# NVlabs/curobo

Measured on NVIDIA B200. Metric: rollout_cost_grad_evals_per_sec, higher is better.
Workload: dtype f32

## Files before the change

### curobo_b200/csrc/cb200_blob.h

```cpp
#pragma once
#include <stdint.h>

namespace cb200 {

constexpr int32_t kBlobMagic = 0x30324243;
constexpr int kMaxLinks = 64;

struct BlobHeader {
  int32_t magic;
  int32_t total_bytes;
  int32_t smem_bytes;
  int32_t nl, D, S, L, P;
  int32_t n_levels;
  int32_t off_fixed;
  int32_t off_joff;
  int32_t off_link_map;
  int32_t off_joint_map;
  int32_t off_joint_type;
  int32_t off_tool_map;
  int32_t off_spheres;
  int32_t off_sph_link;
  int32_t off_padding;
  int32_t off_link_sph_off;
  int32_t off_link_sph_idx;
  int32_t off_level_off;
  int32_t off_level_links;
  int32_t off_anc_mask;
  int32_t off_jl_off;
  int32_t off_jl_idx;
  int32_t off_limits;
  int32_t off_pairs;
  int32_t n_cl, n_lp;
  int32_t off_cl_link;
  int32_t off_cl_start;
  int32_t off_cl_bound;
  int32_t off_lp;
  int32_t n_fk_steps;
  int32_t off_fk_sched;
  int32_t off_cl_bound_scene;
  int32_t off_sph_cl;
  int32_t n_sphere_cfgs;
  int32_t reserved[10];
};
static_assert(sizeof(BlobHeader) == 192, "BlobHeader must be 192 bytes");

}
```

### curobo_b200/csrc/cb200_kernels.cu

```cuda
#include <cuda_runtime.h>
#include <stdio.h>
#include <stdlib.h>
#include <string.h>

#include <algorithm>
#include <cmath>
#include <vector>

#include "../../include/curobo_b200.h"
#include "cb200_blob.h"
#include "cb200_bspline.cuh"
#include "cb200_dynamics.cuh"
#include "cb200_dynamics_tile.cuh"
#include "cb200_launch.h"
#include "cb200_math.cuh"
#include "cb200_mesh.cuh"
#include "cb200_warp.cuh"

using namespace cb200;

namespace {

constexpr int kWarpsPerCta = 8;
#ifndef CB200_MINB
// ... 189 lines not shown
    pg[0] = pg[1] = pg[2] = pg[4] = pg[5] = pg[6] = 0.0f;
    if (do_pose) {
      const int gi = a.idxs_goal ? __ldg(a.idxs_goal + b) : 0;
      const bool term = !(h < a.H - 1 && a.H > 1);
      const float *axes = term ? a.pose_axes_t : a.pose_axes_nt;
      const float *tol = term ? a.pose_tol_t : a.pose_tol_nt;
      const size_t go = ((size_t)gi * L + t) * cfg.num_goalset;
      const PoseOut po = tool_pose_cost(p, qt, a.goal_position + go * 3, a.goal_quat + go * 4, cfg.num_goalset,
                                        cfg.pose_weight[0], cfg.pose_weight[1], axes, t,
                                        tol != nullptr ? __ldg(tol + 2 * t) : 0.0f,
                                        tol != nullptr ? __ldg(tol + 2 * t + 1) : 0.0f, cfg.pose_rotation_method);
      const V3 om = quat_grad_to_omega(qt, po.gq_w, po.gq_x, po.gq_y, po.gq_z);
      pg[0] = po.g_pos.x;
      pg[1] = po.g_pos.y;
      pg[2] = po.g_pos.z;
      pg[4] = om.x;
      pg[5] = om.y;
      pg[6] = om.z;
      pose_c += po.pos_cost + po.rot_cost;
      if (a.pose_cost) {
        a.pose_cost[((size_t)e * L + t) * 2] = po.pos_cost;
        a.pose_cost[((size_t)e * L + t) * 2 + 1] = po.rot_cost;
      }
      if (a.pose_goalset_idx) a.pose_goalset_idx[(size_t)e * L + t] = po.goal_idx;
    }
  }
  __syncwarp();
}

struct RowB1 {
  float self_c, fmax, scene_c;
  int bi, bj, nnz;
};

template <bool SWEEP, int SCENE, bool CULL2 = true>
__device__ __forceinline__ RowB1 row_phase_b1(const FusedArgs &a, const RobotView &rv, const EvalSmem &es, int lane, int e,
                                              int b, const float4 *prev_sph, const float4 *next_sph) {
  const cb200_rollout_cfg &cfg = a.cfg;
  const int S = rv.S;
  RowB1 r{0.0f, 0.0f, 0.0f, 0, 0, 0};
  if (cfg.self_weight > 0.0f && rv.P > 0) {
    r.fmax = (rv.n_lp > 0) ? warp_self_collision_tiles<true, CULL2>(rv, es, lane, r.bi, r.bj)
                           : warp_self_collision_pairs(es.gsph, rv.pairs, rv.P, lane, r.bi, r.bj);
    r.self_c = (r.fmax > 0.0f) ? 0.5f * cfg.self_weight * r.fmax : 0.0f;
  }
  if (a.self_cost && lane == 0) a.self_cost[e] = r.self_c;
  __syncwarp();
  const bool do_scene = SCENE != 0 && cfg.scene_weight > 0.0f;
  const int env = (a.env_query_idx != nullptr) ? __ldg(a.env_query_idx + b) : 0;
  const float sdt = (SWEEP && cfg.use_speed_metric && (a.dt != nullptr || a.spl.knots != nullptr))
                        ? (a.spl.knots != nullptr ? __ldg(a.spl.traj_dt + __ldg(a.spl.goal_idx)) : __ldg(a.dt))
                        : 0.0f;
  int ce = 0, ncub = 0;
  bool cull = false;
  if ((SCENE & 1) && do_scene) {
    ce = env < a.cuboids.num_envs ? env : 0;
    ncub = a.cuboids.count[ce];
    if (ncub > a.cuboids.max_n) ncub = a.cuboids.max_n;
    cull = !SWEEP && rv.n_lp > 0 && ncub <= 32;
    if (cull) {
#pragma unroll 1
      for (int ca = lane; ca < rv.n_cl; ca += 32) {
        const float4 cb = rv.cl_bound_scene[ca];
        uint32_t mask = 0u;
        if (cb.w >= 0.0f) {
          const float *Tk = es.cumul + 12 * rv.cl_link[ca];
          const V3 cw = mk3(Tk[0] * cb.x + Tk[1] * cb.y + Tk[2] * cb.z + Tk[3], Tk[4] * cb.x + Tk[5] * cb.y + Tk[6] * cb.z + Tk[7],
                            Tk[8] * cb.x + Tk[9] * cb.y + Tk[10] * cb.z + Tk[11]);
#pragma unroll 1
          for (int i = 0; i < ncub; ++i) {
            const int kk = ce * a.cuboids.max_n + i;
            if (a.cuboids.enable[kk] != 1) continue;
            const ObsFrame f = load_obs_frame(a.cuboids.inv_pose + 8 * kk);
            const SdfGrad sg = cuboid_sdf_grad(to_obstacle(f, cw), ldgf(a.cuboids.dims + 4 * kk), ldgf(a.cuboids.dims + 4 * kk + 1),
                                               ldgf(a.cuboids.dims + 4 * kk + 2));
            if (sg.sdf < cb.w + cfg.scene_activation) mask |= (1u << i);
          }
        }
        es.cmask[ca] = mask;
      }
      __syncwarp();
    }
  }
#pragma unroll 1
  for (int s = lane; s < S; s += 32) {
    V3 g = mk3(0, 0, 0);
    float c = 0.0f;
    if (do_scene) {
      const float4 sp = es.sph[s];
      const V3 cen = mk3(sp.x, sp.y, sp.z);
      if (!SWEEP) {
        if (sp.w >= 0.0f) {
          if (SCENE & 1) {
            uint32_t m = cull ? es.cmask[rv.sph_cl[s]] : 0xffffffffu;
            const float radj = sp.w + cfg.scene_activation;
#pragma unroll 1
            for (int i = 0; i < ncub && m != 0u; ++i) {
              if (cull && !((m >> i) & 1u)) continue;
              if (cull) m &= ~(1u << i);
              const int kk = ce * a.cuboids.max_n + i;
              if (a.cuboids.enable[kk] != 1) continue;
              const ObsFrame f = load_obs_frame(a.cuboids.inv_pose + 8 * kk);
              const SdfGrad sg = cuboid_sdf_grad(to_obstacle(f, cen), ldgf(a.cuboids.dims + 4 * kk), ldgf(a.cuboids.dims + 4 * kk + 1),
                                                 ldgf(a.cuboids.dims + 4 * kk + 2));
              const float pen = radj - sg.sdf;
              if (pen > 0.0f) {
                float ac, as;
                collision_activation(pen, cfg.scene_activation, ac, as);
                c += cfg.scene_weight * ac;
                g = g + (cfg.scene_weight * as) * from_obstacle(f, sg.n);
              }
            }
          }
          if (SCENE & 2) {
            const CuboidSet none{};
            c += sphere_scene_discrete<2>(cen, sp.w, cfg.scene_activation, cfg.scene_weight, none, a.voxels, env, g);
          }
        }
      } else {
        V3 pv = cen, nx = cen;
        if (prev_sph != nullptr) {
          const float4 t = prev_sph[s];
          pv = mk3(t.x, t.y, t.z);
        }
        if (next_sph != nullptr) {
          const float4 t = next_sph[s];
          nx = mk3(t.x, t.y, t.z);
        }
        c = sphere_scene_swept<SCENE>(cen, sp.w, cfg.scene_activation, cfg.scene_weight, prev_sph != nullptr, pv,
                                      next_sph != nullptr, nx, a.cuboids, a.voxels, env, g);
        if (cfg.use_speed_metric && prev_sph != nullptr && next_sph != nullptr) speed_metric(pv, cen, nx, sdt, c, g);
      }
    }
    es.gsph[s] = make_float4(g.x, g.y, g.z, 0.0f);
    r.nnz += (g.x != 0.0f || g.y != 0.0f || g.z != 0.0f) ? 1 : 0;
    r.scene_c += c;
    if (a.scene_cost) a.scene_cost[(size_t)e * S + s] = c;
  }
  __syncwarp();
  r.nnz = (int)__reduce_add_sync(kFull, (unsigned)r.nnz) + 2;
  return r;
}

template <bool SMALL = false>
__device__ __forceinline__ void row_phase_b2(const FusedArgs &a, const RobotView &rv, const EvalSmem &es,
                                             const unsigned char *smem_blob, int lane, int e, const RowB1 &r,
                                             float cs_cost, float pose_c) {
  if (r.fmax > 0.0f && lane == 0) {
    const float4 pi = es.sph[r.bi], pj = es.sph[r.bj];
    const float w = a.cfg.self_weight;
    float4 gi = es.gsph[r.bi], gj = es.gsph[r.bj];
    const float gx = w * (pj.x - pi.x), gy = w * (pj.y - pi.y), gz = w * (pj.z - pi.z);
    gi.x += gx;
    gi.y += gy;
    gi.z += gz;
    gj.x -= gx;
    gj.y -= gy;
    gj.z -= gz;
    es.gsph[r.bi] = gi;
    es.gsph[r.bj] = gj;
  }
  __syncwarp();
  float *gq = a.grad_q + (size_t)e * rv.D;
  if (!warp_fk_backward_sparse<SMALL>(rv, es, lane, gq, r.nnz)) warp_fk_backward_cold(smem_blob, a.blob, es.cumul, lane, gq);
  const float tot = warp_sum(cs_cost + pose_c + r.scene_c) + r.self_c;
  if (lane == 0) a.cost[e] = tot;
  __syncwarp();
}

#ifdef CB200_OOL_PHASES
struct PhaseAOut {
  float cs_cost, pose_c;
};
static __device__ __noinline__ PhaseAOut phase_a_ool(const FusedArgs *a, const unsigned char *smem, float *base, int lane,
                                                     int e, int b, int h) {
  const RobotView rv = make_robot_view(smem, a->blob);
  const EvalSmem es = carve_eval_smem(base, rv.nl, rv.D, rv.S, rv.L, rv.n_cl);
  PhaseAOut o;
  row_phase_a<false>(*a, rv, es, lane, e, b, h, o.cs_cost, o.pose_c);
  return o;
}
template <int SCENE>
static __device__ __noinline__ RowB1 phase_b1_ool(const FusedArgs *a, const unsigned char *smem, float *base, int lane, int e,
                                                  int b) {
  const RobotView rv = make_robot_view(smem, a->blob);
  const EvalSmem es = carve_eval_smem(base, rv.nl, rv.D, rv.S, rv.L, rv.n_cl);
  return row_phase_b1<false, SCENE>(*a, rv, es, lane, e, b, nullptr, nullptr);
}
static __device__ __noinline__ void phase_b2_ool(const FusedArgs *a, const unsigned char *smem, float *base, int lane, int e,
                                                 RowB1 r, float cs_cost, float pose_c) {
  const RobotView rv = make_robot_view(smem, a->blob);
  const EvalSmem es = carve_eval_smem(base, rv.nl, rv.D, rv.S, rv.L, rv.n_cl);
  row_phase_b2(*a, rv, es, smem, lane, e, r, cs_cost, pose_c);
}
#endif

template <int SCENE, bool SPLINE, int MINB = CB200_MINB>
__global__ void __launch_bounds__(kWarpsPerCta * 32, MINB) rollout_fused_kernel(const __grid_constant__ FusedArgs a) {
  CB200_EXTERN_SHARED __align__(128) unsigned char smem[];
  __shared__ unsigned long long mbar;
  stage_blob_to_smem(smem, a.blob, (uint32_t)a.blob_smem_bytes, &mbar);
  const int warp = threadIdx.x >> 5, lane = threadIdx.x & 31, nwarps = blockDim.x >> 5;
  float *base = reinterpret_cast<float *>(smem + a.blob_smem_bytes) + (size_t)warp * a.eval_floats;
  const int N = a.B * a.H;
  const int stride = gridDim.x * nwarps;
  int e = blockIdx.x * nwarps + warp;
  while (e < N) {
    int b = e, h = 0;
    if (a.H != 1) {
      b = e / a.H;
      h = e - b * a.H;
    }
#ifndef CB200_OOL_PHASES
    const RobotView rv = make_robot_view(smem, a.blob);
    const EvalSmem es = carve_eval_smem(base, rv.nl, rv.D, rv.S, rv.L, rv.n_cl);
    float cs_cost = 0.0f, pose_c = 0.0f;
    row_phase_a<SPLINE>(a, rv, es, lane, e, b, h, cs_cost, pose_c);
    const RowB1 r = row_phase_b1<false, SCENE, MINB != 3>(a, rv, es, lane, e, b, nullptr, nullptr);
    row_phase_b2<MINB == 3>(a, rv, es, smem, lane, e, r, cs_cost, pose_c);
#else
    const PhaseAOut pa = phase_a_ool(&a, smem, base, lane, e, b, h);
    const RowB1 r = phase_b1_ool<SCENE>(&a, smem, base, lane, e, b);
    phase_b2_ool(&a, smem, base, lane, e, r, pa.cs_cost, pa.pose_c);
#endif
    if (a.work_counter != nullptr) {
      int nxt = 0;
      if (lane == 0) nxt = stride + atomicAdd(a.work_counter, 1);
      e = __shfl_sync(kFull, nxt, 0);
    } else {
      e += stride;
    }
  }
  if (a.work_counter != nullptr && lane == 0) {
    __threadfence();
    if (atomicAdd(a.work_counter + 1, 1) == stride - 1) {
      a.work_counter[0] = 0;
      a.work_counter[1] = 0;
    }
  }
}

constexpr int kBigWarps = 16;

template <int SCENE, bool SMALL = false>
__device__ __forceinline__ RowB1 row_phase_b1_list(const FusedArgs &a, const RobotView &rv, const EvalSmem &es, int lane, int e,
                                                   int b, int &n_list, bool &dense) {
  const cb200_rollout_cfg &cfg = a.cfg;
  const int S = rv.S;
  RowB1 r{0.0f, 0.0f, 0.0f, 0, 0, 0};
  n_list = 0;
  dense = false;
  if (cfg.self_weight > 0.0f && rv.P > 0) {
    r.fmax = warp_self_collision_tiles<false, !SMALL>(rv, es, lane, r.bi, r.bj);
    r.self_c = (r.fmax > 0.0f) ? 0.5f * cfg.self_weight * r.fmax : 0.0f;
  }
  if (a.self_cost && lane == 0) a.self_cost[e] = r.self_c;
  __syncwarp();
  const bool do_scene = SCENE != 0 && cfg.scene_weight > 0.0f;
  const int env = (a.env_query_idx != nullptr) ? __ldg(a.env_query_idx + b) : 0;
  int ce = 0, ncub = 0;
  bool cull = false;
  if ((SCENE & 1) && do_scene) {
    ce = env < a.cuboids.num_envs ? env : 0;
    ncub = a.cuboids.count[ce];
    if (ncub > a.cuboids.max_n) ncub = a.cuboids.max_n;
    cull = rv.n_lp > 0 && ncub <= 32;
    if (cull) {
#pragma unroll 1
      for (int ca = lane; ca < rv.n_cl; ca += 32) {
        const float4 cb = rv.cl_bound_scene[ca];
        uint32_t mask = 0u;
        if (cb.w >= 0.0f) {
          const float *Tk = es.cumul + 12 * rv.cl_link[ca];
          const V3 cw = mk3(Tk[0] * cb.x + Tk[1] * cb.y + Tk[2] * cb.z + Tk[3], Tk[4] * cb.x + Tk[5] * cb.y + Tk[6] * cb.z + Tk[7],
                            Tk[8] * cb.x + Tk[9] * cb.y + Tk[10] * cb.z + Tk[11]);
#pragma unroll 1
          for (int i = 0; i < ncub; ++i) {
            const int kk = ce * a.cuboids.max_n + i;
            if (a.cuboids.enable[kk] != 1) continue;
            const ObsFrame f = load_obs_frame(a.cuboids.inv_pose + 8 * kk);
            const SdfGrad sg = cuboid_sdf_grad(to_obstacle(f, cw), ldgf(a.cuboids.dims + 4 * kk), ldgf(a.cuboids.dims + 4 * kk + 1),
                                               ldgf(a.cuboids.dims + 4 * kk + 2));
            if (sg.sdf < cb.w + cfg.scene_activation) mask |= (1u << i);
          }
        }
        es.cmask[ca] = mask;
      }
      __syncwarp();
    }
  }
  bool ft_live = false;
  const unsigned lt = (1u << lane) - 1u;
#pragma unroll 1
  for (int base = 0; base < S; base += 32) {
    const int s = base + lane;
    V3 g = mk3(0, 0, 0);
    float c = 0.0f;
// ... 2142 lines not shown
  h->S = S;
  h->L = L;
  h->P = P;
  h->n_levels = n_levels;
  h->off_fixed = take((int64_t)nl * 48);
  h->off_joff = take((int64_t)nl * 8);
  h->off_link_map = take((int64_t)nl * 2);
  h->off_joint_map = take((int64_t)nl * 2);
  h->off_joint_type = take(nl);
  h->off_tool_map = take((int64_t)L * 2);
  h->off_spheres = take((int64_t)S * 16);
  h->off_sph_link = take((int64_t)S * 2);
  h->off_padding = take((int64_t)S * 4);
  h->off_link_sph_off = take((int64_t)(nl + 1) * 2);
  h->off_link_sph_idx = take((int64_t)S * 2);
  h->off_level_off = take((int64_t)(nl + 1) * 2);
  h->off_level_links = take((int64_t)nl * 2);
  h->off_anc_mask = take((int64_t)nl * 8);
  h->off_jl_off = take((int64_t)(D + 1) * 2);
  h->off_jl_idx = take((int64_t)nl * 2);
  h->off_limits = take((int64_t)10 * D * 4);
  const int max_cl = std::min(nl, S);
  h->off_cl_link = take((int64_t)max_cl * 2);
  h->off_cl_start = take((int64_t)(max_cl + 1) * 2);
  h->off_cl_bound = take((int64_t)max_cl * 16);
  h->off_lp = take((int64_t)n_lp_cap * 4);
  h->off_fk_sched = take((int64_t)nl * 8);
  h->off_cl_bound_scene = take((int64_t)max_cl * 16);
  h->off_sph_cl = take((int64_t)S);
  h->smem_bytes = (int32_t)off;
  h->off_pairs = take((int64_t)P * 4);
  h->total_bytes = (int32_t)off;
  return off;
}

static int lp_cap(const cb200_robot_sizes *sz) {
  const int m = std::min(sz->num_links, sz->num_spheres);
  return std::min(m * (m - 1) / 2, std::max(sz->num_pairs, 0));
}

int cb200_voxel_mip_block(void) { return kMipBlock; }

int64_t cb200_voxel_mip_stride(const float *host_params, int num_layers) {
  if (host_params == nullptr || num_layers < 1) return -1;
  int64_t best = 1;
  for (int k = 0; k < num_layers; ++k) {
    const int64_t nx = (int64_t)host_params[4 * k], ny = (int64_t)host_params[4 * k + 1], nz = (int64_t)host_params[4 * k + 2];
    best = std::max(best, ((nx + kMipBlock - 1) >> kMipShift) * ((ny + kMipBlock - 1) >> kMipShift) * ((nz + kMipBlock - 1) >> kMipShift));
  }
  return best;
}

int cb200_voxel_build_mip(const cb200_voxel_set *vs, cb200_stream_t stream) {
  CB200_DEVICE_GUARD((vs != nullptr ? vs->mip : nullptr));
  if (vs == nullptr || vs->mip == nullptr || vs->mip_stride < 1 || vs->features == nullptr || vs->params == nullptr ||
      vs->max_n < 1 || vs->num_envs < 1)
    return ret(cudaErrorInvalidValue);
  const int n_layers = vs->max_n * vs->num_envs;
  const long long n = (long long)vs->mip_stride * n_layers;
  const int grid = (int)std::min<long long>((n + 127) / 128, 148LL * 16);
  CB200_LAUNCH(voxel_mip_kernel, grid, 128, 0, (cudaStream_t)stream, to_dev(vs), const_cast<uint16_t *>(vs->mip), n_layers);
  return launch_status();
}

int64_t cb200_robot_blob_bytes(const cb200_robot_sizes *sz) {
  BlobHeader h;
  return blob_layout(sz, nullptr, &h, lp_cap(sz));
}

int64_t cb200_pack_robot_blob(void *out, int64_t out_bytes, const cb200_robot_sizes *sz, const float *fixed_transforms,
                              const int16_t *link_map, const int16_t *joint_map, const int8_t *joint_map_type,
                              const float *joint_offset_map, const int16_t *tool_frame_map, const float *link_spheres,
                              const int16_t *link_sphere_map, const float *sphere_padding,
                              const int16_t *collision_pairs, const float *position_limits,
                              const float *velocity_limits, const float *acceleration_limits, const float *jerk_limits,
                              const float *effort_limits) {
  BlobHeader h;
  const int64_t total = blob_layout(sz, link_map, &h, lp_cap(sz));
  if (total < 0) return total;
  if (out_bytes < total) return -3;
  const int nl = h.nl, D = h.D, S = h.S, L = h.L, P = h.P;
  const int n_cfg = sz->num_sphere_configs > 1 ? sz->num_sphere_configs : 1;
  h.n_sphere_cfgs = n_cfg;
  unsigned char *o = static_cast<unsigned char *>(out);
  memset(o, 0, (size_t)total);
  memcpy(o, &h, sizeof(h));
  memcpy(o + h.off_fixed, fixed_transforms, (size_t)nl * 48);
  memcpy(o + h.off_joff, joint_offset_map, (size_t)nl * 8);
  memcpy(o + h.off_link_map, link_map, (size_t)nl * 2);
  memcpy(o + h.off_joint_map, joint_map, (size_t)nl * 2);
  memcpy(o + h.off_joint_type, joint_map_type, (size_t)nl);
  if (L) memcpy(o + h.off_tool_map, tool_frame_map, (size_t)L * 2);
  for (int l = 0; l < nl; ++l) {
    const int jt = joint_map_type[l];
    if (jt < -1 || jt > 5) return -4;
    if (jt >= 0 && (joint_map[l] < 0 || joint_map[l] >= D)) return -5;
  }
  for (int t = 0; t < L; ++t)
    if (tool_frame_map[t] < 0 || tool_frame_map[t] >= nl) return -6;
  if (S) {
    memcpy(o + h.off_spheres, link_spheres, (size_t)S * 16);
    memcpy(o + h.off_sph_link, link_sphere_map, (size_t)S * 2);
    memcpy(o + h.off_padding, sphere_padding, (size_t)S * 4);
  }
  int16_t *lso = reinterpret_cast<int16_t *>(o + h.off_link_sph_off);
  int16_t *lsi = reinterpret_cast<int16_t *>(o + h.off_link_sph_idx);
  int n = 0;
  for (int l = 0; l < nl; ++l) {
    lso[l] = (int16_t)n;
    for (int s = 0; s < S; ++s) {
      if (link_sphere_map[s] < 0 || link_sphere_map[s] >= nl) return -7;
      if (link_sphere_map[s] == l) lsi[n++] = (int16_t)s;
    }
  }
  lso[nl] = (int16_t)n;
  std::vector<int> depth(nl, 0);
  unsigned long long *anc = reinterpret_cast<unsigned long long *>(o + h.off_anc_mask);
  anc[0] = 1ull;
  for (int l = 1; l < nl; ++l) {
    depth[l] = depth[link_map[l]] + 1;
    anc[l] = anc[link_map[l]] | (1ull << l);
  }
  int16_t *lvo = reinterpret_cast<int16_t *>(o + h.off_level_off);
  int16_t *lvl = reinterpret_cast<int16_t *>(o + h.off_level_links);
  n = 0;
  for (int lev = 0; lev < h.n_levels; ++lev) {
    lvo[lev] = (int16_t)n;
    for (int l = 0; l < nl; ++l)
      if (depth[l] == lev) lvl[n++] = (int16_t)l;
  }
  lvo[h.n_levels] = (int16_t)n;
  {
    uint32_t *sched = reinterpret_cast<uint32_t *>(o + h.off_fk_sched);
    int steps = 0;
    for (int lev = 1; lev < h.n_levels; ++lev) {
      for (int i = lvo[lev]; i < lvo[lev + 1]; i += 2) {
        const uint32_t l0 = (uint32_t)lvl[i], p0 = (uint32_t)link_map[l0];
        sched[2 * steps] = (l0 * 48u) | ((p0 * 48u) << 16);
        sched[2 * steps + 1] = 0xffffu;
        if (i + 1 < lvo[lev + 1]) {
          const uint32_t l1 = (uint32_t)lvl[i + 1], p1 = (uint32_t)link_map[l1];
          sched[2 * steps + 1] = (l1 * 48u) | ((p1 * 48u) << 16);
        }
        ++steps;
      }
    }
    reinterpret_cast<BlobHeader *>(o)->n_fk_steps = steps;
  }
  int16_t *jlo = reinterpret_cast<int16_t *>(o + h.off_jl_off);
  int16_t *jli = reinterpret_cast<int16_t *>(o + h.off_jl_idx);
  n = 0;
  for (int d = 0; d < D; ++d) {
    jlo[d] = (int16_t)n;
    for (int l = 0; l < nl; ++l)
      if (joint_map_type[l] >= 0 && joint_map[l] == d) jli[n++] = (int16_t)l;
  }
  jlo[D] = (int16_t)n;
  float *lim = reinterpret_cast<float *>(o + h.off_limits);
  const float *srcs[5] = {position_limits, velocity_limits, acceleration_limits, jerk_limits, effort_limits};
  for (int k = 0; k < 5; ++k)
    for (int i = 0; i < 2 * D; ++i) lim[k * 2 * D + i] = srcs[k] ? srcs[k][i] : (i < D ? -1e30f : 1e30f);
  for (int p = 0; p < P; ++p) {
    const int i = collision_pairs[2 * p], j = collision_pairs[2 * p + 1];
    if (i < 0 || j < 0 || i >= S || j >= S) return -8;
  }
  if (P) memcpy(o + h.off_pairs, collision_pairs, (size_t)P * 4);
// ... 508 lines not shown
```

### curobo_b200/csrc/cb200_warp.cuh

```cuda
#pragma once
#include "cb200_blob.h"
#include "cb200_math.cuh"

namespace cb200 {

constexpr unsigned kFull = 0xffffffffu;

struct RobotView {
  int nl, D, S, L, P, n_levels;
  const float *fixed;
  const float *joff;
  const int16_t *link_map;
  const int16_t *joint_map;
  const int8_t *joint_type;
  const int16_t *tool_map;
  const float4 *spheres;
  const int16_t *sph_link;
  const float *padding;
  const int16_t *link_sph_off;
  const int16_t *link_sph_idx;
  const int16_t *level_off;
  const int16_t *level_links;
  const unsigned long long *anc_mask;
  const int16_t *jl_off;
  const int16_t *jl_idx;
  const float *limits;
  const uint32_t *pairs;
  int n_cl, n_lp;
  const int16_t *cl_link;
  const int16_t *cl_start;
  const float4 *cl_bound;
  const uint32_t *lp;
  int n_fk_steps;
  const uint32_t *fk_sched;
  const float4 *cl_bound_scene;
  const uint8_t *sph_cl;
};

__device__ __forceinline__ RobotView make_robot_view(const unsigned char *smem_blob, const unsigned char *gmem_blob) {
  const BlobHeader *h = reinterpret_cast<const BlobHeader *>(smem_blob);
  RobotView v;
  v.nl = h->nl;
  v.D = h->D;
  v.S = h->S;
  v.L = h->L;
  v.P = h->P;
  v.n_levels = h->n_levels;
  v.fixed = reinterpret_cast<const float *>(smem_blob + h->off_fixed);
  v.joff = reinterpret_cast<const float *>(smem_blob + h->off_joff);
  v.link_map = reinterpret_cast<const int16_t *>(smem_blob + h->off_link_map);
  v.joint_map = reinterpret_cast<const int16_t *>(smem_blob + h->off_joint_map);
  v.joint_type = reinterpret_cast<const int8_t *>(smem_blob + h->off_joint_type);
  v.tool_map = reinterpret_cast<const int16_t *>(smem_blob + h->off_tool_map);
  v.spheres = reinterpret_cast<const float4 *>(smem_blob + h->off_spheres);
  v.sph_link = reinterpret_cast<const int16_t *>(smem_blob + h->off_sph_link);
  v.padding = reinterpret_cast<const float *>(smem_blob + h->off_padding);
  v.link_sph_off = reinterpret_cast<const int16_t *>(smem_blob + h->off_link_sph_off);
  v.link_sph_idx = reinterpret_cast<const int16_t *>(smem_blob + h->off_link_sph_idx);
  v.level_off = reinterpret_cast<const int16_t *>(smem_blob + h->off_level_off);
  v.level_links = reinterpret_cast<const int16_t *>(smem_blob + h->off_level_links);
  v.anc_mask = reinterpret_cast<const unsigned long long *>(smem_blob + h->off_anc_mask);
  v.jl_off = reinterpret_cast<const int16_t *>(smem_blob + h->off_jl_off);
  v.jl_idx = reinterpret_cast<const int16_t *>(smem_blob + h->off_jl_idx);
  v.limits = reinterpret_cast<const float *>(smem_blob + h->off_limits);
  v.pairs = reinterpret_cast<const uint32_t *>(gmem_blob + h->off_pairs);
  v.n_cl = h->n_cl;
  v.n_lp = h->n_lp;
  v.cl_link = reinterpret_cast<const int16_t *>(smem_blob + h->off_cl_link);
  v.cl_start = reinterpret_cast<const int16_t *>(smem_blob + h->off_cl_start);
  v.cl_bound = reinterpret_cast<const float4 *>(smem_blob + h->off_cl_bound);
  v.lp = reinterpret_cast<const uint32_t *>(smem_blob + h->off_lp);
  v.n_fk_steps = h->n_fk_steps;
  v.fk_sched = reinterpret_cast<const uint32_t *>(smem_blob + h->off_fk_sched);
  v.cl_bound_scene = reinterpret_cast<const float4 *>(smem_blob + h->off_cl_bound_scene);
  v.sph_cl = reinterpret_cast<const uint8_t *>(smem_blob + h->off_sph_cl);
  return v;
}

struct EvalSmem {
  float *cumul;
  float4 *sph;
  float4 *gsph;
  float *ft;
  float *contrib;
  float *qv;
  float *gqv;
  float *pose_g;
  float4 *bc;
  uint32_t *cmask;
  float4 *glist;
};
__host__ __device__ inline int eval_smem_floats(int nl, int D, int S, int L, int n_cl) {
  int n = nl * 12 + S * 8 + nl * 8 + n_cl * 4;
  n += nl + D + D + L * 8 + n_cl;
  return (n + 3) & ~3;
}
__device__ __forceinline__ EvalSmem carve_eval_smem(float *base, int nl, int D, int S, int L, int n_cl) {
  EvalSmem e;
  e.cumul = base;
  e.sph = reinterpret_cast<float4 *>(base + nl * 12);
  e.gsph = e.sph + S;
  e.ft = base + nl * 12 + S * 8;
  e.bc = reinterpret_cast<float4 *>(e.ft + nl * 8);
  e.contrib = e.ft + nl * 8 + n_cl * 4;
  e.qv = e.contrib + nl;
  e.gqv = e.qv + D;
  e.pose_g = e.gqv + D;
  e.cmask = reinterpret_cast<uint32_t *>(e.pose_g + L * 8);
  e.glist = nullptr;
  return e;
}

constexpr int kGradListCap = 96;
__host__ __device__ inline int big_smem_floats(int nl, int D, int S, int L, int n_cl) {
  int n = nl * 12 + S * 4 + nl * 8 + n_cl * 4 + kGradListCap * 4;
  n += nl + D + D + L * 8 + n_cl;
  return (n + 3) & ~3;
}
__device__ __forceinline__ EvalSmem carve_big_smem(float *base, int nl, int D, int S, int L, int n_cl) {
  EvalSmem e;
  e.cumul = base;
  e.sph = reinterpret_cast<float4 *>(base + nl * 12);
  e.gsph = nullptr;
  e.ft = base + nl * 12 + S * 4;
  e.bc = reinterpret_cast<float4 *>(e.ft + nl * 8);
  e.glist = e.bc + n_cl;
  e.contrib = reinterpret_cast<float *>(e.glist + kGradListCap);
  e.qv = e.contrib + nl;
  e.gqv = e.qv + D;
  e.pose_g = e.gqv + D;
  e.cmask = reinterpret_cast<uint32_t *>(e.pose_g + L * 8);
  return e;
}

__device__ __forceinline__ float warp_sum(float v) {
#pragma unroll
  for (int o = 16; o > 0; o >>= 1) v += __shfl_xor_sync(kFull, v, o);
  return v;
}

__device__ __forceinline__ void warp_fk_compose(const RobotView &rv, const EvalSmem &es, int lane);
__device__ __forceinline__ void warp_fk(const RobotView &rv, const EvalSmem &es, int lane) {
  const bool scratch = rv.S * 4 >= rv.nl * 12;
  float *loc = scratch ? reinterpret_cast<float *>(es.sph) : es.cumul;
  #pragma unroll 1
  for (int l = lane; l < rv.nl; l += 32) {
    int jt = rv.joint_type[l];
    float th = 0.0f;
    if (jt >= 0) th = rv.joff[2 * l] * es.qv[rv.joint_map[l]] + rv.joff[2 * l + 1];
    local_link_transform(rv.fixed + 12 * l, jt, th, (l == 0 ? es.cumul : loc) + 12 * l);
  }
  __syncwarp();
  warp_fk_compose(rv, es, lane);
}

__device__ __forceinline__ void warp_fk_compose(const RobotView &rv, const EvalSmem &es, int lane) {
  const bool scratch = rv.S * 4 >= rv.nl * 12;
  const float *loc = scratch ? reinterpret_cast<const float *>(es.sph) : es.cumul;
  const int sub = lane >> 4, k = lane & 15;
  const bool lane_ok = k < 12;
  const uint32_t row_off = (uint32_t)(k >> 2) * 16u, col_off = (uint32_t)(k & 3) * 4u, k_off = (uint32_t)k * 4u;
  const float cw = ((k & 3) == 3) ? 1.0f : 0.0f;
  unsigned char *cumb = reinterpret_cast<unsigned char *>(es.cumul);
  const unsigned char *locb = reinterpret_cast<const unsigned char *>(loc);
#pragma unroll 1
  for (int st = 0; st < rv.n_fk_steps; ++st) {
    const uint32_t w = rv.fk_sched[2 * st + sub];
    const uint32_t l_off = w & 0xffffu, p_off = w >> 16;
    const bool act = lane_ok && (l_off != 0xffffu);
    float out = 0.0f;
    if (act) {
      const float4 pr = *reinterpret_cast<const float4 *>(cumb + p_off + row_off);
      const float *Lm = reinterpret_cast<const float *>(locb + l_off + col_off);
      out = pr.x * Lm[0] + pr.y * Lm[4] + pr.z * Lm[8] + cw * pr.w;
    }
    if (!scratch) __syncwarp();
    if (act) *reinterpret_cast<float *>(cumb + l_off + k_off) = out;
    __syncwarp();
  }
}

__device__ __forceinline__ void warp_spheres(const RobotView &rv, const EvalSmem &es, int lane, float4 *out_global,
                                             const float4 *cfg_spheres = nullptr) {
  #pragma unroll 1
  for (int s = lane; s < rv.S; s += 32) {
    const float *T = es.cumul + 12 * rv.sph_link[s];
    const float4 p = cfg_spheres != nullptr ? __ldg(cfg_spheres + s) : rv.spheres[s];
    const float4 r0 = *reinterpret_cast<const float4 *>(T), r1 = *reinterpret_cast<const float4 *>(T + 4),
                 r2 = *reinterpret_cast<const float4 *>(T + 8);
    float4 w;
    w.x = r0.x * p.x + r0.y * p.y + r0.z * p.z + r0.w;
    w.y = r1.x * p.x + r1.y * p.y + r1.z * p.z + r1.w;
    w.z = r2.x * p.x + r2.y * p.y + r2.z * p.z + r2.w;
    w.w = p.w;
    es.sph[s] = w;
    if (out_global != nullptr) out_global[s] = w;
    if (es.gsph != nullptr) {
      w.w = p.w + rv.padding[s];
      es.gsph[s] = w;
    }
  }
}

__device__ __forceinline__ float warp_self_collision_pairs(const float4 *psph, const uint32_t *pairs, int P, int lane,
                                                           int &bi, int &bj) {
  float best = 0.0f;
  uint32_t best_p = 0xffffffffu;
  #pragma unroll 1
  for (int p = lane; p < P; p += 32) {
    const uint32_t pr = __ldg(pairs + p);
    const float4 a = psph[pr & 0xffffu], b = psph[pr >> 16];
    const float rs = a.w + b.w;
    const float dx = a.x - b.x, dy = a.y - b.y, dz = a.z - b.z;
    float f = rs * rs - (dx * dx + dy * dy + dz * dz);
    if (!(a.w >= 0.0f && b.w >= 0.0f)) f = 0.0f;
    if (f > best) {
      best = f;
      best_p = (uint32_t)p;
    }
  }
  const uint32_t fb = __reduce_max_sync(kFull, __float_as_uint(best));
  const uint32_t cand = (__float_as_uint(best) == fb && best > 0.0f) ? best_p : 0xffffffffu;
  const uint32_t win = __reduce_min_sync(kFull, cand);
  bi = bj = 0;
  if (win == 0xffffffffu) return 0.0f;
  const uint32_t pr = __ldg(pairs + win);
  bi = (int)(pr & 0xffffu);
  bj = (int)(pr >> 16);
  return __uint_as_float(fb);
}

template <bool PADDED_COPY>
__device__ __forceinline__ float4 padded_sphere(const RobotView &rv, const EvalSmem &es, int i) {
  if (PADDED_COPY) return es.gsph[i];
  float4 x = es.sph[i];
  x.w += rv.padding[i];
  return x;
}

template <bool PADDED_COPY = true, bool CULL2 = true>
__device__ __forceinline__ float warp_self_collision_tiles(const RobotView &rv, const EvalSmem &es, int lane, int &bi,
                                                           int &bj, int base0 = 0, int stride = 32,
                                                           unsigned char *idx_scratch = nullptr,
                                                           unsigned long long *key_out = nullptr, bool fill_bounds = true) {
  if (fill_bounds) {
    #pragma unroll 1
    for (int a = lane; a < rv.n_cl; a += 32) {
      const float4 c = rv.cl_bound[a];
      const float *T = es.cumul + 12 * rv.cl_link[a];
      es.bc[a] = make_float4(T[0] * c.x + T[1] * c.y + T[2] * c.z + T[3], T[4] * c.x + T[5] * c.y + T[6] * c.z + T[7],
                             T[8] * c.x + T[9] * c.y + T[10] * c.z + T[11], c.w);
    }
    __syncwarp();
  }
  unsigned long long key = 0ull;
  #pragma unroll 1
  for (int base = base0; base < rv.n_lp; base += stride) {
    uint32_t pr = 0;
    bool hit = false;
    if (base + lane < rv.n_lp) {
      pr = rv.lp[base + lane];
      const float4 A = es.bc[pr & 0xffffu], B = es.bc[pr >> 16];
      const float dx = A.x - B.x, dy = A.y - B.y, dz = A.z - B.z, rs = A.w + B.w;
      hit = (A.w >= 0.0f) && (B.w >= 0.0f) && (dx * dx + dy * dy + dz * dz < rs * rs);
    }
    unsigned m = __ballot_sync(kFull, hit);
    while (m) {
      const int src = __ffs(m) - 1;
// ... 70 lines not shown
  bj = 0xffff - (int)(key & 0xffffu);
  return __uint_as_float((uint32_t)(key >> 32));
}

__device__ __forceinline__ void warp_fk_upsweep(const RobotView &rv, const EvalSmem &es, int lane, float *gq_out);
__device__ __forceinline__ void warp_fk_backward(const RobotView &rv, const EvalSmem &es, int lane, float *gq_out) {
  #pragma unroll 1
  for (int k = lane; k < rv.nl; k += 32) {
    const float *Tk = es.cumul + 12 * k;
    const V3 o = mk3(Tk[3], Tk[7], Tk[11]);
    V3 F = mk3(0, 0, 0), T = mk3(0, 0, 0);
    #pragma unroll 1
    for (int i = rv.link_sph_off[k]; i < rv.link_sph_off[k + 1]; ++i) {
      const int s = rv.link_sph_idx[i];
      const float4 g4 = es.gsph[s];
      const V3 g = mk3(g4.x, g4.y, g4.z);
      if (g.x == 0.0f && g.y == 0.0f && g.z == 0.0f) continue;
      const float4 p4 = es.sph[s];
      F = F + g;
      T = T + cross(mk3(p4.x, p4.y, p4.z) - o, g);
    }
    for (int e = 0; e < rv.L; ++e) {
      if (rv.tool_map[e] != k) continue;
      F = F + mk3(es.pose_g[8 * e + 0], es.pose_g[8 * e + 1], es.pose_g[8 * e + 2]);
      T = T + mk3(es.pose_g[8 * e + 4], es.pose_g[8 * e + 5], es.pose_g[8 * e + 6]);
    }
    float *ft = es.ft + 8 * k;
    ft[0] = F.x;
    ft[1] = F.y;
    ft[2] = F.z;
    ft[4] = T.x;
    ft[5] = T.y;
    ft[6] = T.z;
  }
  __syncwarp();
  warp_fk_upsweep(rv, es, lane, gq_out);
}

__device__ __forceinline__ void warp_fk_upsweep(const RobotView &rv, const EvalSmem &es, int lane, float *gq_out) {
  #pragma unroll 1
  for (int j = lane; j < rv.nl; j += 32) {
    const int jt = rv.joint_type[j];
    float res = 0.0f;
    if (jt >= 0) {
      const float *Tj = es.cumul + 12 * j;
      const V3 oj = mk3(Tj[3], Tj[7], Tj[11]);
      V3 F = mk3(0, 0, 0), T = mk3(0, 0, 0);
      #pragma unroll 1
      for (int k = j; k < rv.nl; ++k) {
        if (!((rv.anc_mask[k] >> j) & 1ull)) continue;
        const float *ft = es.ft + 8 * k;
        const V3 Fk = mk3(ft[0], ft[1], ft[2]);
        const float *Tk = es.cumul + 12 * k;
        const V3 ok = mk3(Tk[3], Tk[7], Tk[11]);
        F = F + Fk;
        T = T + mk3(ft[4], ft[5], ft[6]) + cross(ok - oj, Fk);
      }
      const int ax = (jt >= JT_XR) ? jt - JT_XR : jt;
      const V3 a = mk3(Tj[ax], Tj[4 + ax], Tj[8 + ax]);
      res = rv.joff[2 * j] * ((jt >= JT_XR) ? dot(a, T) : dot(a, F));
    }
    es.contrib[j] = res;
  }
  __syncwarp();
  for (int d = lane; d < rv.D; d += 32) {
    float g = es.gqv[d];
    for (int i = rv.jl_off[d]; i < rv.jl_off[d + 1]; ++i) g += es.contrib[rv.jl_idx[i]];
    gq_out[d] = g;
  }
}

static __device__ __noinline__ void warp_fk_backward_cold(const unsigned char *smem_blob, const unsigned char *gmem_blob,
                                                          float *eval_base, int lane, float *gq_out) {
  const RobotView rv = make_robot_view(smem_blob, gmem_blob);
  const EvalSmem es = carve_eval_smem(eval_base, rv.nl, rv.D, rv.S, rv.L, rv.n_cl);
  warp_fk_backward(rv, es, lane, gq_out);
}

template <bool SMALL = false>
__device__ __forceinline__ bool warp_fk_backward_sparse(const RobotView &rv, const EvalSmem &es, int lane, float *gq_out,
                                                        int nnz) {
  if (nnz > 2 * rv.nl) return false;
  if (SMALL) {
    float sc = 0.0f;
    V3 ax = mk3(0, 0, 0), og = mk3(0, 0, 0);
    int jt = -1;
    if (lane < rv.nl) {
      jt = rv.joint_type[lane];
      if (jt >= 0) {
        const float *Tj = es.cumul + 12 * lane;
        const int a = (jt >= JT_XR) ? jt - JT_XR : jt;
        ax = mk3(Tj[a], Tj[4 + a], Tj[8 + a]);
        og = mk3(Tj[3], Tj[7], Tj[11]);
        sc = rv.joff[2 * lane];
      }
    }
    float acc = 0.0f;
    const int n_entries = rv.S + rv.L;
#pragma unroll 1
    for (int base = 0; base < n_entries; base += 32) {
      const int s = base + lane;
      bool nz = false;
      if (s < rv.S) {
        const float4 g = es.gsph[s];
        nz = (g.x != 0.0f) || (g.y != 0.0f) || (g.z != 0.0f);
      } else if (s < n_entries) {
        const float *pg = es.pose_g + 8 * (s - rv.S);
        nz = pg[0] != 0.0f || pg[1] != 0.0f || pg[2] != 0.0f || pg[4] != 0.0f || pg[5] != 0.0f || pg[6] != 0.0f;
      }
      unsigned m = __ballot_sync(kFull, nz);
      while (m) {
        const int ss = base + __ffs(m) - 1;
        m &= m - 1;
        V3 p, g, om = mk3(0, 0, 0);
        int k;
        if (ss < rv.S) {
          const float4 g4 = es.gsph[ss], p4 = es.sph[ss];
          k = rv.sph_link[ss];
          p = mk3(p4.x, p4.y, p4.z);
          g = mk3(g4.x, g4.y, g4.z);
        } else {
          const float *pg = es.pose_g + 8 * (ss - rv.S);
          k = rv.tool_map[ss - rv.S];
          const float *Tk = es.cumul + 12 * k;
          p = mk3(Tk[3], Tk[7], Tk[11]);
          g = mk3(pg[0], pg[1], pg[2]);
          om = mk3(pg[4], pg[5], pg[6]);
        }
        if (jt >= 0 && ((rv.anc_mask[k] >> lane) & 1ull))
          acc += (jt >= JT_XR) ? sc * (dot(ax, cross(p - og, g)) + dot(ax, om)) : sc * dot(ax, g);
      }
    }
    if (lane < rv.nl) es.contrib[lane] = acc;
    __syncwarp();
    for (int d = lane; d < rv.D; d += 32) {
      float g = es.gqv[d];
      for (int i = rv.jl_off[d]; i < rv.jl_off[d + 1]; ++i) g += es.contrib[rv.jl_idx[i]];
      gq_out[d] = g;
    }
    return true;
  }
  const int nu = rv.nl > 32 ? 2 : 1;
  V3 ax[2], og[2];
  float sc[2];
  int jt[2];
#pragma unroll
  for (int u = 0; u < 2; ++u) {
    const int j = lane + 32 * u;
    jt[u] = -1;
    if (u >= nu) continue;
    sc[u] = 0.0f;
    ax[u] = og[u] = mk3(0, 0, 0);
    if (j < rv.nl) {
      jt[u] = rv.joint_type[j];
      if (jt[u] >= 0) {
        const float *Tj = es.cumul + 12 * j;
        const int a = (jt[u] >= JT_XR) ? jt[u] - JT_XR : jt[u];
        ax[u] = mk3(Tj[a], Tj[4 + a], Tj[8 + a]);
        og[u] = mk3(Tj[3], Tj[7], Tj[11]);
        sc[u] = rv.joff[2 * j];
      }
    }
  }
  float acc[2] = {0.0f, 0.0f};
  auto add = [&](unsigned long long mask, V3 p, V3 g, V3 om) {
#pragma unroll
    for (int u = 0; u < 2; ++u) {
      const int j = lane + 32 * u;
      if (u < nu && jt[u] >= 0 && ((mask >> j) & 1ull)) {
        acc[u] += (jt[u] >= JT_XR) ? sc[u] * (dot(ax[u], cross(p - og[u], g)) + dot(ax[u], om)) : sc[u] * dot(ax[u], g);
      }
    }
  };
  #pragma unroll 1
  for (int base = 0; base < rv.S; base += 32) {
    const int s = base + lane;
    bool nz = false;
    if (s < rv.S) {
      const float4 g = es.gsph[s];
      nz = (g.x != 0.0f) || (g.y != 0.0f) || (g.z != 0.0f);
    }
    unsigned m = __ballot_sync(kFull, nz);
    while (m) {
      const int ss = base + __ffs(m) - 1;
      m &= m - 1;
      const float4 g4 = es.gsph[ss], p4 = es.sph[ss];
      add(rv.anc_mask[rv.sph_link[ss]], mk3(p4.x, p4.y, p4.z), mk3(g4.x, g4.y, g4.z), mk3(0, 0, 0));
    }
  }
  #pragma unroll 1
  for (int t = 0; t < rv.L; ++t) {
    const float *pg = es.pose_g + 8 * t;
    const V3 g = mk3(pg[0], pg[1], pg[2]), om = mk3(pg[4], pg[5], pg[6]);
    if (g.x == 0.0f && g.y == 0.0f && g.z == 0.0f && om.x == 0.0f && om.y == 0.0f && om.z == 0.0f) continue;
    const int k = rv.tool_map[t];
    const float *Tk = es.cumul + 12 * k;
    add(rv.anc_mask[k], mk3(Tk[3], Tk[7], Tk[11]), g, om);
  }
#pragma unroll
  for (int u = 0; u < 2; ++u) {
    const int j = lane + 32 * u;
    if (j < rv.nl) es.contrib[j] = acc[u];
  }
  __syncwarp();
  for (int d = lane; d < rv.D; d += 32) {
    float g = es.gqv[d];
    for (int i = rv.jl_off[d]; i < rv.jl_off[d + 1]; ++i) g += es.contrib[rv.jl_idx[i]];
    gq_out[d] = g;
  }
  return true;
}

__device__ __forceinline__ void warp_zero_ft(const RobotView &rv, const EvalSmem &es, int lane) {
  for (int k = lane; k < rv.nl * 2; k += 32) reinterpret_cast<float4 *>(es.ft)[k] = make_float4(0.f, 0.f, 0.f, 0.f);
  __syncwarp();
}
__device__ __forceinline__ void warp_drain_list_to_ft(const RobotView &rv, const EvalSmem &es, int lane, int n) {
#pragma unroll 1
  for (int i = 0; i < n; ++i) {
    const float4 g4 = es.glist[i];
    const int s = __float_as_int(g4.w);
    const float4 p4 = es.sph[s];
    const int k = rv.sph_link[s];
    const float *Tk = es.cumul + 12 * k;
    const V3 g = mk3(g4.x, g4.y, g4.z);
    const V3 tq = cross(mk3(p4.x - Tk[3], p4.y - Tk[7], p4.z - Tk[11]), g);
    if (lane < 6) {
      const float v = lane == 0 ? g.x : lane == 1 ? g.y : lane == 2 ? g.z : lane == 3 ? tq.x : lane == 4 ? tq.y : tq.z;
      es.ft[8 * k + lane + (lane >= 3 ? 1 : 0)] += v;
    }
    __syncwarp();
  }
}
__device__ __forceinline__ void warp_fk_backward_from_ft(const RobotView &rv, const EvalSmem &es, int lane, float *gq_out) {
  if (lane == 0) {
    for (int t = 0; t < rv.L; ++t) {
      float *ft = es.ft + 8 * rv.tool_map[t];
      const float *pg = es.pose_g + 8 * t;
      ft[0] += pg[0];
      ft[1] += pg[1];
      ft[2] += pg[2];
      ft[4] += pg[4];
      ft[5] += pg[5];
      ft[6] += pg[6];
    }
  }
  __syncwarp();
  warp_fk_upsweep(rv, es, lane, gq_out);
}
__device__ __forceinline__ void warp_list_accumulate(const RobotView &rv, const EvalSmem &es, int lane, const float4 *list, int n,
                                                     bool with_tools, float (&acc)[2]) {
  const int nu = rv.nl > 32 ? 2 : 1;
  V3 ax[2], og[2];
  float sc[2];
  int jt[2];
#pragma unroll
  for (int u = 0; u < 2; ++u) {
    const int j = lane + 32 * u;
    jt[u] = -1;
    if (u >= nu) continue;
    sc[u] = 0.0f;
// ... 191 lines not shown
```

Before: 232.5 million.

## Skip trailing disabled spheres and split sparse joint-gradient loop across half-warps

Computes at pack time the index past the last sphere with non-negative radius (S_act). Sphere transform, scene-cost and backward loops then stop at S_act, with tail gradients pre-set once per warp and tail scene costs written as zero. For robots with at most 16 links, the sparse backward accumulation also has each half-warp take a different nonzero entry per iteration and combines the halves with a shuffle, halving the serial iterations. This relies on the disabled-tail assumption holding when no per-call sphere overrides are given, and it adds branching.

```diff
diff --git a/curobo_b200/csrc/cb200_blob.h b/curobo_b200/csrc/cb200_blob.h
--- a/curobo_b200/csrc/cb200_blob.h
+++ b/curobo_b200/csrc/cb200_blob.h
@@ -40,7 +40,8 @@
   int32_t off_cl_bound_scene;
   int32_t off_sph_cl;
   int32_t n_sphere_cfgs;
-  int32_t reserved[10];
+  int32_t S_act;
+  int32_t reserved[9];
 };
 static_assert(sizeof(BlobHeader) == 192, "BlobHeader must be 192 bytes");
 
diff --git a/curobo_b200/csrc/cb200_kernels.cu b/curobo_b200/csrc/cb200_kernels.cu
--- a/curobo_b200/csrc/cb200_kernels.cu
+++ b/curobo_b200/csrc/cb200_kernels.cu
@@ -295,8 +295,10 @@
       __syncwarp();
     }
   }
+  if (a.scene_cost != nullptr)
+    for (int s = rv.S_act + lane; s < S; s += 32) a.scene_cost[(size_t)e * S + s] = 0.0f;
 #pragma unroll 1
-  for (int s = lane; s < S; s += 32) {
+  for (int s = lane; s < rv.S_act; s += 32) {
     V3 g = mk3(0, 0, 0);
     float c = 0.0f;
     if (do_scene) {
@@ -408,6 +410,16 @@
 }
 #endif
 
+__device__ __forceinline__ int init_disabled_sphere_tail(const FusedArgs &a, const unsigned char *smem_blob, float *base,
+                                                         int lane) {
+  const BlobHeader *h = reinterpret_cast<const BlobHeader *>(smem_blob);
+  if (a.sphere_cfgs != nullptr || a.robot_spheres != nullptr) return h->S;
+  const EvalSmem es = carve_eval_smem(base, h->nl, h->D, h->S, h->L, h->n_cl);
+  for (int s = h->S_act + lane; s < h->S; s += 32) es.gsph[s] = make_float4(0.0f, 0.0f, 0.0f, -1.0f);
+  __syncwarp();
+  return h->S_act;
+}
+
 template <int SCENE, bool SPLINE, int MINB = CB200_MINB>
 __global__ void __launch_bounds__(kWarpsPerCta * 32, MINB) rollout_fused_kernel(const __grid_constant__ FusedArgs a) {
   CB200_EXTERN_SHARED __align__(128) unsigned char smem[];
@@ -417,6 +429,7 @@
   float *base = reinterpret_cast<float *>(smem + a.blob_smem_bytes) + (size_t)warp * a.eval_floats;
   const int N = a.B * a.H;
   const int stride = gridDim.x * nwarps;
+  const int S_act = init_disabled_sphere_tail(a, smem, base, lane);
   int e = blockIdx.x * nwarps + warp;
   while (e < N) {
     int b = e, h = 0;
@@ -425,7 +438,8 @@
       h = e - b * a.H;
     }
 #ifndef CB200_OOL_PHASES
-    const RobotView rv = make_robot_view(smem, a.blob);
+    RobotView rv = make_robot_view(smem, a.blob);
+    rv.S_act = S_act;
     const EvalSmem es = carve_eval_smem(base, rv.nl, rv.D, rv.S, rv.L, rv.n_cl);
     float cs_cost = 0.0f, pose_c = 0.0f;
     row_phase_a<SPLINE>(a, rv, es, lane, e, b, h, cs_cost, pose_c);
@@ -2734,6 +2748,9 @@
   const int nl = h.nl, D = h.D, S = h.S, L = h.L, P = h.P;
   const int n_cfg = sz->num_sphere_configs > 1 ? sz->num_sphere_configs : 1;
   h.n_sphere_cfgs = n_cfg;
+  h.S_act = 0;
+  for (int s = 0; s < S; ++s)
+    if (link_spheres[4 * s + 3] >= 0.0f || link_spheres[4 * s + 3] + sphere_padding[s] >= 0.0f) h.S_act = s + 1;
   unsigned char *o = static_cast<unsigned char *>(out);
   memset(o, 0, (size_t)total);
   memcpy(o, &h, sizeof(h));
diff --git a/curobo_b200/csrc/cb200_warp.cuh b/curobo_b200/csrc/cb200_warp.cuh
--- a/curobo_b200/csrc/cb200_warp.cuh
+++ b/curobo_b200/csrc/cb200_warp.cuh
@@ -8,6 +8,7 @@
 
 struct RobotView {
   int nl, D, S, L, P, n_levels;
+  int S_act;
   const float *fixed;
   const float *joff;
   const int16_t *link_map;
@@ -43,6 +44,7 @@
   v.nl = h->nl;
   v.D = h->D;
   v.S = h->S;
+  v.S_act = h->S;
   v.L = h->L;
   v.P = h->P;
   v.n_levels = h->n_levels;
@@ -183,7 +185,7 @@
 __device__ __forceinline__ void warp_spheres(const RobotView &rv, const EvalSmem &es, int lane, float4 *out_global,
                                              const float4 *cfg_spheres = nullptr) {
   #pragma unroll 1
-  for (int s = lane; s < rv.S; s += 32) {
+  for (int s = lane; s < rv.S_act; s += 32) {
     const float *T = es.cumul + 12 * rv.sph_link[s];
     const float4 p = cfg_spheres != nullptr ? __ldg(cfg_spheres + s) : rv.spheres[s];
     const float4 r0 = *reinterpret_cast<const float4 *>(T), r1 = *reinterpret_cast<const float4 *>(T + 4),
@@ -420,55 +422,66 @@
                                                         int nnz) {
   if (nnz > 2 * rv.nl) return false;
   if (SMALL) {
+    const bool halves = rv.nl <= 16;
+    const int j = halves ? (lane & 15) : lane;
+    const unsigned pair_mask = halves ? ~0u : 0u;
+    const bool upper = halves && lane >= 16;
     float sc = 0.0f;
     V3 ax = mk3(0, 0, 0), og = mk3(0, 0, 0);
     int jt = -1;
-    if (lane < rv.nl) {
-      jt = rv.joint_type[lane];
+    if (j < rv.nl) {
+      jt = rv.joint_type[j];
       if (jt >= 0) {
-        const float *Tj = es.cumul + 12 * lane;
+        const float *Tj = es.cumul + 12 * j;
         const int a = (jt >= JT_XR) ? jt - JT_XR : jt;
         ax = mk3(Tj[a], Tj[4 + a], Tj[8 + a]);
         og = mk3(Tj[3], Tj[7], Tj[11]);
-        sc = rv.joff[2 * lane];
+        sc = rv.joff[2 * j];
       }
     }
     float acc = 0.0f;
-    const int n_entries = rv.S + rv.L;
+    const int S = rv.S_act, n_entries = S + rv.L;
 #pragma unroll 1
     for (int base = 0; base < n_entries; base += 32) {
       const int s = base + lane;
       bool nz = false;
-      if (s < rv.S) {
+      if (s < S) {
         const float4 g = es.gsph[s];
         nz = (g.x != 0.0f) || (g.y != 0.0f) || (g.z != 0.0f);
       } else if (s < n_entries) {
-        const float *pg = es.pose_g + 8 * (s - rv.S);
+        const float *pg = es.pose_g + 8 * (s - S);
         nz = pg[0] != 0.0f || pg[1] != 0.0f || pg[2] != 0.0f || pg[4] != 0.0f || pg[5] != 0.0f || pg[6] != 0.0f;
       }
       unsigned m = __ballot_sync(kFull, nz);
       while (m) {
-        const int ss = base + __ffs(m) - 1;
+        int bit = __ffs(m) - 1;
         m &= m - 1;
+        const unsigned m1 = m & pair_mask;
+        const int bit1 = __ffs(m1) - 1;
+        m &= ~(m1 & (0u - m1));
+        if (upper) bit = bit1;
+        if (bit < 0) continue;
+        const int ss = base + bit;
         V3 p, g, om = mk3(0, 0, 0);
         int k;
-        if (ss < rv.S) {
+        if (ss < S) {
           const float4 g4 = es.gsph[ss], p4 = es.sph[ss];
           k = rv.sph_link[ss];
           p = mk3(p4.x, p4.y, p4.z);
           g = mk3(g4.x, g4.y, g4.z);
         } else {
-          const float *pg = es.pose_g + 8 * (ss - rv.S);
-          k = rv.tool_map[ss - rv.S];
+          const float *pg = es.pose_g + 8 * (ss - S);
+          k = rv.tool_map[ss - S];
           const float *Tk = es.cumul + 12 * k;
           p = mk3(Tk[3], Tk[7], Tk[11]);
           g = mk3(pg[0], pg[1], pg[2]);
           om = mk3(pg[4], pg[5], pg[6]);
         }
-        if (jt >= 0 && ((rv.anc_mask[k] >> lane) & 1ull))
+        if (jt >= 0 && ((rv.anc_mask[k] >> j) & 1ull))
           acc += (jt >= JT_XR) ? sc * (dot(ax, cross(p - og, g)) + dot(ax, om)) : sc * dot(ax, g);
       }
     }
+    if (halves) acc += __shfl_xor_sync(kFull, acc, 16);
     if (lane < rv.nl) es.contrib[lane] = acc;
     __syncwarp();
     for (int d = lane; d < rv.D; d += 32) {
@@ -511,10 +524,10 @@
     }
   };
   #pragma unroll 1
-  for (int base = 0; base < rv.S; base += 32) {
+  for (int base = 0; base < rv.S_act; base += 32) {
     const int s = base + lane;
     bool nz = false;
-    if (s < rv.S) {
+    if (s < rv.S_act) {
       const float4 g = es.gsph[s];
       nz = (g.x != 0.0f) || (g.y != 0.0f) || (g.z != 0.0f);
     }
```

Result: faster. 241.6 million (median of 6 runs) (+3.9%).
